# oiwn/toy-heaan-ckks

Measured on AMD Instinct MI355X. Metric: RNS-NTT poly-muls/sec (N=2^16, 16 primes) at 1/2/4/8 GPUs; % HBM roofline, higher is better.
Workload: dtype u32

## Files before the change

toy-heaan-ckks_amd/csrc/rnt_mfma.hip:

```cpp
#include <hip/hip_runtime.h>

#include <vector>

#include "rnt_internal.hpp"
#include "rnt_hostmath.hpp"
#include "rnt_modarith.hpp"
#include "rnt_device.hpp"

namespace rnt {

#ifdef RNT_MF_TRACE
constexpr int kMfTraceWg = 4096, kMfTraceSt = 16;
__device__ uint64_t g_mf_trace[kMfTraceWg * 16 * kMfTraceSt];
#define MF_STAMP(S)                                                                                  \
  do {                                                                                               \
    const uint32_t wg_ = blockIdx.x + blockIdx.y * gridDim.x;                                        \
    if ((threadIdx.x & 63u) == 0 && wg_ < (uint32_t)kMfTraceWg)                                      \
      g_mf_trace[(wg_ * 16 + (threadIdx.x >> 6)) * kMfTraceSt + (S)] = __builtin_amdgcn_s_memrealtime(); \
  } while (0)
#else
#define MF_STAMP(S) \
  do {              \
  } while (0)
#endif

namespace mf {

typedef int v4i __attribute__((ext_vector_type(4)));
constexpr int kT = 1024;
constexpr uint32_t kN = 1u << 16;
constexpr uint32_t K32 = 0x80808080u;

constexpr int S_F1 = 0, S_F2 = 1, S_F3 = 17, S_F4 = 18, S_I4 = 19, S_I3 = 20, S_I2 = 21, S_I1 = 37;
constexpr int kSlots = 38;
constexpr int kMat = 0;
constexpr int kCompF1 = kSlots * 4 * 64;
constexpr int kCompI4 = kCompF1 + 64;
constexpr int kTw3f = kCompI4 + 64;
constexpr int kTw4f = kTw3f + 1024;
constexpr int kTw4i = kTw4f + 16384;
constexpr int kTw3i = kTw4i + 16384;
constexpr int S_F4S = (kTw3i + 1024 + 255) / 256;
#ifndef RNT_MF_FOLD3
#define RNT_MF_FOLD3 1
#endif
#ifndef RNT_MF_FOLD4
#define RNT_MF_FOLD4 0
#endif
constexpr bool kFold3 = RNT_MF_FOLD3 != 0, kFold4 = RNT_MF_FOLD4 != 0;
constexpr int kFoldBase = (S_F4S + 1) * 256;
constexpr int kTwB3 = 1024, kTwB4 = 16384;
constexpr int kTw3fA = kFoldBase, kTw3iA = kTw3fA + 2 * kTwB3;
constexpr int kFold4Base = kFoldBase + (kFold3 ? 4 * kTwB3 : 0);
constexpr int kTw4fA = kFold4Base, kTw4iA = kTw4fA + 2 * kTwB4;
#ifndef RNT_MF_QR
#define RNT_MF_QR 3
#endif
#ifndef RNT_MF_QR_MUL
#define RNT_MF_QR_MUL RNT_MF_QR
#endif
#ifndef RNT_MF_QR_NTT
#define RNT_MF_QR_NTT RNT_MF_QR
#endif
#ifndef RNT_MF_QR_NTTF
#define RNT_MF_QR_NTTF (RNT_MF_QR & 1)
#endif
#ifndef RNT_MF_QR_TENSOR
#define RNT_MF_QR_TENSOR RNT_MF_QR
#endif
constexpr int kQrMul = RNT_MF_QR_MUL & 3, kQrNtt = RNT_MF_QR_NTT & 3, kQrNttFwd = RNT_MF_QR_NTTF & 3;
constexpr int kQrTensor = RNT_MF_QR_TENSOR & 3;
constexpr bool kQrAny = (kQrMul | kQrNtt | kQrNttFwd | kQrTensor) != 0;
constexpr int kQrP4 = 4;
constexpr int kQrBase = kFold4Base + (kFold4 ? 4 * kTwB4 : 0);
static_assert(kQrBase % 256 == 0, "matrix slots are 256 v4i");
constexpr int S_QF1 = kQrBase / 256, S_QF3 = S_QF1 + 1, S_QF4 = S_QF1 + 2, S_QI4 = S_QF1 + 3, S_QI2 = S_QF1 + 4;
constexpr int kQCompF1 = (S_QI2 + 16) * 256, kQCompI4 = kQCompF1 + 128;
constexpr int kQConst = kQCompI4 + 128;
constexpr int kQrEnd = kQConst + 64;
constexpr int kLimb = kQrAny ? kQrEnd : kQrBase;
static_assert(!kQrAny || (kQConst < kLimb && (S_QI2 + 16) * 256 <= kQCompF1), "the plain slots lie inside the limb's table");
#define RNT_MF_QRC "48"
constexpr uint32_t kQrC = 48;
constexpr int kTw3iR = kFold3 ? kTw3iA : kTw3i;
constexpr int kTw4fR = kFold4 ? kTw4fA : kTw4f, kTw4iR = kFold4 ? kTw4iA : kTw4i;
constexpr bool kFold3Fwd = false;
constexpr size_t kLdsBytes = (size_t)160 * 1024;
static_assert(kLdsBytes > 80 * 1024, "one workgroup per CU");

__host__ __device__ constexpr int p3(int c, int i) {
  return 4 * (8 * (i >> 1) + 4 * (i & 1) + 2 * ((c >> 1) & 1) + (c & 1)) + 2 * (c >> 3) + ((c >> 2) & 1);
}
__host__ __device__ constexpr int q2(int c, int i) {
  return p3(8 * (i >> 1) + 4 * (i & 1) + 2 * (c >> 3) + ((c >> 2) & 1), 2 * ((c >> 1) & 1) + (c & 1));
}

struct Mc {
  int32_t q;
  uint32_t nqinv;
  int64_t K;
  int64_t K0;
  int32_t one;
  int32_t s16;
  int32_t mu;
  uint32_t nq, kq, kq0;
};

typedef __amdgpu_buffer_rsrc_t Rsrc;
__device__ __forceinline__ Rsrc rsrc(const void* base, uint32_t bytes) {
  return __builtin_amdgcn_make_buffer_rsrc((void*)base, 0, (int)bytes, 0x00020000);
}
#ifndef RNT_MF_NT
#define RNT_MF_NT 2
#endif
constexpr int kStreamAux = RNT_MF_NT;
#ifndef RNT_MF_LAST_NT
#define RNT_MF_LAST_NT 2
#endif
constexpr int kLastAux = RNT_MF_LAST_NT;
template <int AUX = 0>
__device__ __forceinline__ v4i bld(Rsrc r, uint32_t voff, uint32_t soff) {
  const auto v = __builtin_amdgcn_raw_buffer_load_b128(r, voff, soff, AUX);
  return v4i{(int)v[0], (int)v[1], (int)v[2], (int)v[3]};
}
template <int AUX = 0>
__device__ __forceinline__ void bst(v4i x, Rsrc r, uint32_t voff, uint32_t soff) {
  using V4 = decltype(__builtin_amdgcn_raw_buffer_load_b128(r, 0, 0, 0));
  V4 v;
  v[0] = (uint32_t)x[0];
  v[1] = (uint32_t)x[1];
  v[2] = (uint32_t)x[2];
  v[3] = (uint32_t)x[3];
  __builtin_amdgcn_raw_buffer_store_b128(v, r, voff, soff, AUX);
  asm volatile("s_nop 1" ::"v"(v));
}

template <bool WK>
__device__ __forceinline__ int32_t recomb(int32_t c0, int32_t c1, int32_t c2, int32_t c3, const Mc& m) {
  const int32_t lo = c0 + (int32_t)((uint32_t)c1 << 8);
  const int32_t hi = c2 + (int32_t)((uint32_t)c3 << 8);
  int64_t t;
  if constexpr (WK) {
    uint64_t cc;
    asm("v_mad_i64_i32 %0, %1, %2, 1, %3" : "=v"(t), "=s"(cc) : "v"(lo), "s"(m.K));
  } else {
    t = (int64_t)lo;
  }
  t = (int64_t)hi * m.s16 + t;
  const uint32_t mm = (uint32_t)t * m.nqinv;
  const int64_t v = (int64_t)(int32_t)mm * m.q + t;
  return (int32_t)(v >> 32);
}
template <bool WK>
__device__ __forceinline__ int32_t recomb_q(int32_t c0, int32_t c1, int32_t c2, int32_t c3, const Mc& m) {
  uint32_t lo = (uint32_t)c0 + ((uint32_t)c1 << 8);
  uint32_t hi = (uint32_t)c2 + ((uint32_t)c3 << 8);
  asm("" : "+v"(lo), "+v"(hi));
  uint32_t t = (hi << 16) + lo;
  asm("" : "+v"(t));
  const int32_t qt = __mulhi((int32_t)hi, m.mu);
  return (int32_t)(t + (uint32_t)qt * m.nq + (WK ? m.kq : m.kq0));
}
template <bool QR, bool WK>
__device__ __forceinline__ int32_t recomb_x(int32_t c0, int32_t c1, int32_t c2, int32_t c3, const Mc& m) {
// ... 529 lines not shown
  return (((uint32_t)i << 14) | ((uint32_t)(hc & 1) << 10) | ((uint32_t)(hc >> 1) << 7)) * 4u;
}
__device__ __forceinline__ void load_p1(uint32_t (&x1)[64], Rsrc src, const Th& h) {
  const uint32_t lo = p1_lane(h), wo = p1_wave(h);
#pragma unroll
  for (int hc = 0; hc < 4; ++hc)
#pragma unroll
    for (int i = 0; i < 4; ++i) {
      const v4i v = bld<kStreamAux>(src, lo, wo + p1_reg(i, hc));
#pragma unroll
      for (int e = 0; e < 4; ++e) x1[4 * (4 * hc + e) + i] = (uint32_t)v[e];
    }
}
template <int C0>
__device__ __forceinline__ void ipass_p1(uint32_t (&x1)[64], const v4i (&M)[4], const Mc& m, Rsrc dst,
                                         const Th& h) {
  const v4i z = {0, 0, 0, 0};
#pragma unroll
  for (int c = C0; c < C0 + 8; ++c) {
    v4i b;
#pragma unroll
    for (int i = 0; i < 4; ++i) b[i] = (int)x1[4 * c + i];
    v4i D[4];
    tile<false, false>(D, M, b, z);
#pragma unroll
    for (int i = 0; i < 4; ++i) x1[4 * c + i] = canon(recomb<false>(D[0][i], D[1][i], D[2][i], D[3][i], m), m.q);
    if ((c & 3) == 3) {
      const int hc = c >> 2;
      const uint32_t lo = p1_lane(h), wo = p1_wave(h);
#pragma unroll
      for (int i = 0; i < 4; ++i) {
        v4i v;
#pragma unroll
        for (int e = 0; e < 4; ++e) v[e] = (int)x1[4 * (4 * hc + e) + i];
        bst<kStreamAux>(v, dst, lo, wo + p1_reg(i, hc));
      }
    } else {
      pin4(x1[4 * c + 0], x1[4 * c + 1], x1[4 * c + 2], x1[4 * c + 3]);
    }
    tile_fence();
  }
}

__device__ __forceinline__ uint32_t p4_lane(const Th& h) { return ((h.n() << 4) | (h.g() << 2)) * 4u; }
__device__ __forceinline__ uint32_t p4_soff(const Th& h, int c) { return ((h.w << 12) | ((uint32_t)c << 8)) * 4u; }

struct Tabs {
  Rsrc tab;
  Mc m;
};
__device__ __forceinline__ Tabs tabs_of(const void* mf, const LimbConst<uint32_t>& lc, uint32_t l) {
  Tabs r;
  r.tab = rsrc((const v4i*)mf + (size_t)l * kLimb, (uint32_t)kLimb * 16u);
  r.m.q = (int32_t)lc.q;
  r.m.nqinv = 0u - lc.qinv;
  int64_t K = (int64_t)((uint64_t)K32 << 32), K0 = 0;
  int32_t one = 1, s16 = 65536;
  asm volatile("" : "+s"(one), "+s"(s16), "+s"(K), "+s"(K0));
  if constexpr (kQrAny) {
    int32_t mu = ((const int32_t*)((const v4i*)mf + (size_t)l * kLimb + kQConst))[0];
    uint32_t nq = 0u - lc.q, kq = K32 - (kQrC << 24), kq0 = 0u - (kQrC << 24);
    asm volatile("" : "+s"(mu), "+s"(nq), "+s"(kq), "+s"(kq0));
    r.m.mu = mu;
    r.m.nq = nq;
    r.m.kq = kq;
    r.m.kq0 = kq0;
  }
  r.m.K = K;
  r.m.K0 = K0;
  r.m.one = one;
  r.m.s16 = s16;
  return r;
}

struct NoEpi {
  __device__ void operator()(int, const int32_t (&)[4], uint32_t (&)[64]) const {}
};
template <int NPARK, uint32_t PBASE, uint32_t PSTRIDE>
__device__ __forceinline__ uint32_t park_addr(const uint32_t* lds, const Th& h) {
  static_assert(NPARK * 1024 <= (int)PSTRIDE && PBASE + 16 * PSTRIDE <= kLdsBytes, "park area");
  return (uint32_t)(uintptr_t)lds + PBASE + h.w * PSTRIDE + h.lam() * 16u;
}
template <bool SYNC1, int F4 = S_F4, bool Q4 = false, bool SYNCX = false, int NPARK = 0, uint32_t PBASE = 0,
          uint32_t PSTRIDE = 0, bool F3 = kFold3, int QR = 0, class EPI = NoEpi>
__device__ __forceinline__ void fwd(uint32_t (&x2)[64], Rsrc src, uint32_t* lds, const Th& h, const Tabs& T,
                                    const EPI& epi = EPI{}) {
  const Mc& m = T.m;
  const uint32_t lo = h.lam() * 16u;
  v4i M[4];
  constexpr bool Q1 = (QR & 1) != 0, Q3 = (QR & 2) != 0, Q4P = (QR & kQrP4) != 0;
  load_mat(M, T.tab, Q1 ? S_QF1 : S_F1, lo);
  const v4i comp = bld(T.tab, lo, (uint32_t)(Q1 ? kQCompF1 : kCompF1) * 16u);
  const v4i comp2 = Q1 ? bld(T.tab, lo, (uint32_t)(kQCompF1 + 64) * 16u) : comp;
  uint32_t x1[64];
  load_p1(x1, src, h);
  MF_STAMP(1);
  pass_p1<0, true, Q1>(x1, M, comp, comp2, m);
  MF_STAMP(2);
  if constexpr (SYNC1) __syncthreads();
  uint32_t wb[4], rb[4];
  const uint32_t t3v = h.g() * 256u, t3s = (uint32_t)((F3 ? kTw3fA : kTw3f) + h.w * 64) * 16u;
  if constexpr (Q4) {
    p1_bases4(wb, h);
    x_write_p1q<0>(x1, lds, wb);
    pass_p1<8, true, Q1>(x1, M, comp, comp2, m);
    __syncthreads();
    p2_bases4(rb, h);
    x_read_p2q<0>(x2, lds, rb);
    __syncthreads();
    p1_bases4(wb, h);
    x_write_p1q<1>(x1, lds, wb);
    __syncthreads();
    p2_bases4(rb, h);
    x_read_p2q<1>(x2, lds, rb);
    __syncthreads();
    p1_bases4(wb, h);
    x_write_p1q<2>(x1, lds, wb);
    load_mat(M, T.tab, S_F2 + h.w, lo);
    pass_p2<0, F3>(x2, M, T.tab, t3v, t3s, m);
    __syncthreads();
    p2_bases4(rb, h);
    x_read_p2q<2>(x2, lds, rb);
    __syncthreads();
    p1_bases4(wb, h);
    x_write_p1q<3>(x1, lds, wb);
    __syncthreads();
    p2_bases4(rb, h);
    x_read_p2q<3>(x2, lds, rb);
  } else {
  p1_bases(wb, h);
  x_write_p1<0>(x1, lds, wb);
  pass_p1<8, true, Q1>(x1, M, comp, comp2, m);
  MF_STAMP(3);
  __syncthreads();
  MF_STAMP(4);
  p2_bases(rb, h);
  x_read_p2<0>(x2, lds, rb);
  __syncthreads();
  MF_STAMP(5);
  p1_bases(wb, h);
  x_write_p1<1>(x1, lds, wb);
  load_mat(M, T.tab, S_F2 + h.w, lo);
  pass_p2<0, F3>(x2, M, T.tab, t3v, t3s, m);
  MF_STAMP(6);
  __syncthreads();
  MF_STAMP(7);
  p2_bases(rb, h);
  x_read_p2<1>(x2, lds, rb);
  }
  if constexpr (SYNCX) __syncthreads();
  static_assert(NPARK == 0 || SYNCX, "the park area is free only past SYNCX");
#pragma unroll
  for (int c = 0; c < NPARK; ++c)
    stash_put(park_addr<NPARK, PBASE, PSTRIDE>(lds, h), c, x2[4 * c], x2[4 * c + 1], x2[4 * c + 2], x2[4 * c + 3]);
  pass_p2<8, F3>(x2, M, T.tab, t3v, t3s, m);
  MF_STAMP(8);
#pragma unroll
  for (int c = 0; c < NPARK; ++c) {
    const v4i v = stash_get(park_addr<NPARK, PBASE, PSTRIDE>(lds, h), c);
#pragma unroll
    for (int i = 0; i < 4; ++i) x2[4 * c + i] = (uint32_t)v[i];
  }
  swap_p2p3(x2);
  load_mat(M, T.tab, Q3 ? S_QF3 : S_F3, lo);
  pass_p3<Q3>(x2, M, T.tab, lo, (uint32_t)(kTw4fR + h.w * 1024) * 16u, m);
  MF_STAMP(9);
  load_mat(M, T.tab, F4, lo);
  pass_p4<Q4P>(x2, M, m, epi);
  MF_STAMP(10);
}

template <bool LOAD, bool PK = false, int QR = 0>
__device__ __forceinline__ void inv_x(uint32_t (&x2)[64], Rsrc pr, uint32_t* lds, const Th& h, const Tabs& T) {
  const Mc& m = T.m;
  const uint32_t lo = h.lam() * 16u;
  v4i M[4];
  constexpr bool Q2 = (QR & 1) != 0, Q4 = (QR & 2) != 0;
  load_mat(M, T.tab, Q4 ? S_QI4 : S_I4, lo);
  const v4i comp = bld(T.tab, lo, (uint32_t)(Q4 ? kQCompI4 : kCompI4) * 16u);
  const v4i comp2 = Q4 && !PK ? bld(T.tab, lo, (uint32_t)(kQCompI4 + 64) * 16u) : comp;
  const uint32_t t4s = (uint32_t)(kTw4iR + h.w * 1024) * 16u;
  const v4i tv0 = bld(T.tab, lo, t4s);
  if constexpr (LOAD) {
#pragma unroll
    for (int cc = 0; cc < 16; ++cc) {
      const v4i v = bld<kStreamAux>(pr, p4_lane(h), p4_soff(h, cc));
#pragma unroll
      for (int i = 0; i < 4; ++i) x2[p3(cc, i)] = (uint32_t)v[i];
    }
  } else {
    __syncthreads();
  }
  ipass_p4<PK, Q4>(x2, M, comp, comp2, tv0, T.tab, lo, t4s, m, lds, h);
  load_mat(M, T.tab, S_I3, lo);
  ipass_p3(x2, M, T.tab, h.g() * 16u, (uint32_t)(kTw3iR + h.w * 64) * 16u, m, lds, h);
  swap_q3p2(x2);
  load_mat(M, T.tab, (Q2 ? S_QI2 : S_I2) + h.w, lo);
  uint32_t wb[4], rb[4];
  uint32_t x1[64];
  ipass_p2<0, Q2>(x2, M, m);
  __syncthreads();
  p2_bases(rb, h);
  x_write_p2<0>(x2, lds, rb);
  ipass_p2<8, Q2>(x2, M, m);
  __syncthreads();
  p1_bases(wb, h);
  x_read_p1<0>(x1, lds, wb);
  __syncthreads();
  p2_bases(rb, h);
  x_write_p2<1>(x2, lds, rb);
  load_mat(M, T.tab, S_I1, lo);
  ipass_p1<0>(x1, M, m, pr, h);
  __syncthreads();
  p1_bases(wb, h);
  x_read_p1<1>(x1, lds, wb);
  ipass_p1<8>(x1, M, m, pr, h);
}
__device__ __forceinline__ void inv(Rsrc pr, uint32_t* lds, const Th& h, const Tabs& T) {
  uint32_t x2[64];
  inv_x<true, false, kQrNtt>(x2, pr, lds, h, T);
}

}

template <bool INV>
__global__ void __launch_bounds__(mf::kT, 1)
k_mf_ntt(uint32_t* __restrict__ data, const void* __restrict__ mft, const LimbConst<uint32_t>* __restrict__ lcs,
         uint64_t ls) {
  using namespace mf;
  extern __shared__ __attribute__((aligned(16))) unsigned char smem_raw[];
  uint32_t* lds = (uint32_t*)smem_raw;
  const Th h(threadIdx.x);
  const uint32_t poly = blockIdx.x, l = blockIdx.y;
  MF_STAMP(0);
  uint32_t* p = data + (uint64_t)l * ls + (uint64_t)poly * kN;
  const Tabs T = tabs_of(mft, lcs[l], l);
  const Rsrc pr = rsrc(p, kN * 4u);
  if constexpr (!INV) {
    uint32_t x[64];
    fwd<false, S_F4, false, false, 0, 0, 0, kFold3 && kFold3Fwd, kQrNttFwd>(x, pr, lds, h, T, [&](int cc, const int32_t (&r)[4], uint32_t (&)[64]) {
      bst<kStreamAux>(v4i{(int)canon(r[0], T.m.q), (int)canon(r[1], T.m.q), (int)canon(r[2], T.m.q), (int)canon(r[3], T.m.q)}, pr,
          p4_lane(h), p4_soff(h, cc));
    });
  } else {
    inv(pr, lds, h, T);
  }
#ifdef RNT_MF_TRACE
  __builtin_amdgcn_s_waitcnt(0);
  MF_STAMP(11);
#endif
}

__global__ void __launch_bounds__(mf::kT, 1)
k_mf_tensor(uint32_t* __restrict__ d0, uint32_t* __restrict__ d1, uint32_t* __restrict__ d2, uint64_t ols,
            const uint32_t* __restrict__ c0, const uint32_t* __restrict__ c1, const uint32_t* __restrict__ c0p,
            const uint32_t* __restrict__ c1p, uint64_t ils, uint32_t* __restrict__ scratch, uint32_t slots,
            const void* __restrict__ mft, const LimbConst<uint32_t>* __restrict__ lcs,
            uint32_t* __restrict__ d2hat) {
  using namespace mf;
  extern __shared__ __attribute__((aligned(16))) unsigned char smem_raw[];
  uint32_t* lds = (uint32_t*)smem_raw;
  const Th h(threadIdx.x);
  const uint32_t poly = blockIdx.x, l = blockIdx.y;
  const uint64_t oo = (uint64_t)l * ols + (uint64_t)poly * kN, io = (uint64_t)l * ils + (uint64_t)poly * kN;
  const LimbConst<uint32_t> lc = lcs[l];
  const Tabs T = tabs_of(mft, lc, l);
  const uint32_t q = lc.q, nqi = T.m.nqinv;
  uint64_t so;
  if (slots) {
    const uint32_t xcc = __builtin_amdgcn_s_getreg((31 << 11) | 20) & 7u;
    const uint32_t cu = (__builtin_amdgcn_s_getreg((31 << 11) | 4) >> 8) & 0xffu;
    so = (uint64_t)((xcc << 8) | cu) << 16;
  } else {
    so = (uint64_t)(poly + l * gridDim.x) << 16;
  }
  const Rsrc R0 = rsrc(d0 + oo, kN * 4u), R1 = rsrc(d1 + oo, kN * 4u), R2 = rsrc(d2 + oo, kN * 4u);
  const Rsrc RS = rsrc(scratch + so, kN * 4u);
  const bool want_hat = d2hat != nullptr;
  const Rsrc RH = rsrc(want_hat ? d2hat + oo : d2 + oo, kN * 4u);
  const uint32_t pl = p4_lane(h);
  auto canon4 = [q](const int32_t (&r)[4]) {
    return v4i{(int)canon(r[0], (int32_t)q), (int)canon(r[1], (int32_t)q), (int)canon(r[2], (int32_t)q),
               (int)canon(r[3], (int32_t)q)};
  };
  auto mmul = [q, nqi](uint32_t a, uint32_t b) {
    const uint64_t t = (uint64_t)a * b;
    const uint32_t mm = (uint32_t)t * nqi;
    const uint32_t r = (uint32_t)((t + (uint64_t)mm * q) >> 32);
    return r >= q ? r - q : r;
  };
  const uint32_t rm = lc.rmod, rmp = lc.rmod_p;
  uint32_t x[64];
  constexpr bool SX = RNT_MF_TENSOR_SYNCX != 0;
  constexpr int NP = SX ? RNT_MF_TENSOR_PARK : 0;
  constexpr uint32_t PB = 128u * 1024u, PS = 2048u;
  constexpr int MEAS = RNT_MF_TENSOR_MEAS;
  fwd<false, S_F4, false, SX, NP, PB, PS, kFold3, kQrTensor>(x, rsrc(c0 + io, kN * 4u), lds, h, T, [&](int cc, const int32_t (&r)[4], uint32_t (&)[64]) {
    if constexpr (MEAS != 3) bst(canon4(r), R1, pl, p4_soff(h, cc));
  });
  fwd<!SX, S_F4, false, SX, NP, PB, PS, kFold3, kQrTensor>(x, rsrc(c1 + io, kN * 4u), lds, h, T, [&](int cc, const int32_t (&r)[4], uint32_t (&)[64]) {
    if constexpr (MEAS != 1) bst(canon4(r), RS, pl, p4_soff(h, cc));
  });
  fwd<!SX, S_F4, false, SX, NP, PB, PS, kFold3, kQrTensor>(x, rsrc(c0p + io, kN * 4u), lds, h, T, [&](int cc, const int32_t (&r)[4], uint32_t (&)[64]) {
    const v4i a0 = MEAS == 3 ? canon4(r) : bld(R1, pl, p4_soff(h, cc));
    const v4i a1 = MEAS == 1 ? canon4(r) : bld(RS, pl, p4_soff(h, cc));
    const v4i b = canon4(r);
    v4i o0, t;
#pragma unroll
    for (int i = 0; i < 4; ++i) {
      o0[i] = (int)mmul((uint32_t)a0[i], (uint32_t)b[i]);
      t[i] = (int)mmul((uint32_t)a1[i], (uint32_t)b[i]);
    }
    bst<kLastAux>(o0, R0, pl, p4_soff(h, cc));
    if constexpr (MEAS != 2) bst(t, R2, pl, p4_soff(h, cc));
  });
  fwd<!SX, S_F4, false, RNT_MF_TENSOR_PARK4 && SX, RNT_MF_TENSOR_PARK4 ? NP : 0, PB, PS, kFold3, kQrTensor>(x, rsrc(c1p + io, kN * 4u), lds, h, T, [&](int cc, const int32_t (&r)[4], uint32_t (&xx)[64]) {
    const v4i b = canon4(r);
    const v4i a0 = MEAS == 3 ? b : bld<kLastAux>(R1, pl, p4_soff(h, cc));
    const v4i a1 = MEAS == 1 ? b : bld<kLastAux>(RS, pl, p4_soff(h, cc));
    const v4i t = MEAS == 2 ? b : bld<kLastAux>(R2, pl, p4_soff(h, cc));
    v4i o1;
#pragma unroll
    for (int i = 0; i < 4; ++i) {
      const uint32_t s = (uint32_t)t[i] + mmul((uint32_t)a0[i], (uint32_t)b[i]);
      o1[i] = (int)(s >= q ? s - q : s);
      const uint32_t m = mmul((uint32_t)a1[i], (uint32_t)b[i]);
      const uint32_t qh = (uint32_t)(((uint64_t)m * rmp) >> 32);
      const uint32_t v = m * rm - qh * q;
      xx[p3(cc, i)] = v >= q ? v - q : v;
    }
    pin4(xx[p3(cc, 0)], xx[p3(cc, 1)], xx[p3(cc, 2)], xx[p3(cc, 3)]);
    bst<kLastAux>(o1, R1, pl, p4_soff(h, cc));
    if (want_hat)
      bst<kLastAux>(v4i{(int)xx[p3(cc, 0)], (int)xx[p3(cc, 1)], (int)xx[p3(cc, 2)], (int)xx[p3(cc, 3)]}, RH, pl,
                    p4_soff(h, cc));
  });
  inv_x<false, false, kQrTensor>(x, R2, lds, h, T);
}

#ifndef RNT_MF_MUL_Q4
#define RNT_MF_MUL_Q4 1
#endif
#ifndef RNT_MF_MUL_NOSYNC1
#define RNT_MF_MUL_NOSYNC1 1
#endif
#ifndef RNT_MF_MUL_PARK
#define RNT_MF_MUL_PARK 4
#endif
#ifndef RNT_MF_MUL_MEAS
#define RNT_MF_MUL_MEAS 0
#endif
#ifndef RNT_MF_SLOT_ST_AUX
#define RNT_MF_SLOT_ST_AUX 0
#endif
#ifndef RNT_MF_MUL_MEAS_SKIP
#define RNT_MF_MUL_MEAS_SKIP (RNT_MF_MUL_MEAS ? 16 - kMulLdsTiles : 0)
#endif
constexpr int kMulLdsTiles = RNT_MF_MUL_Q4 ? 6 : 2;
constexpr uint32_t kMulLdsBase = RNT_MF_MUL_Q4 ? (1u << 14) : (1u << 15);
static_assert(kMulLdsBase * 4 + (size_t)kMulLdsTiles * 16 * 1024 <= mf::kLdsBytes, "in the LDS");
__global__ void __launch_bounds__(mf::kT, 1)
k_mf_mul(uint32_t* c, const uint32_t* a, const uint32_t* b, uint64_t ls, uint32_t* __restrict__ scratch,
         uint32_t slots, const void* __restrict__ mft, const LimbConst<uint32_t>* __restrict__ lcs) {
  using namespace mf;
  extern __shared__ __attribute__((aligned(16))) unsigned char smem_raw[];
  uint32_t* lds = (uint32_t*)smem_raw;
  const Th h(threadIdx.x);
  const uint32_t poly = blockIdx.x, l = blockIdx.y;
  const uint64_t o = (uint64_t)l * ls + (uint64_t)poly * kN;
  const LimbConst<uint32_t> lc = lcs[l];
  const Tabs T = tabs_of(mft, lc, l);
  uint64_t so;
  if (slots) {
    const uint32_t xcc = __builtin_amdgcn_s_getreg((31 << 11) | 20) & 7u;
    const uint32_t cu = (__builtin_amdgcn_s_getreg((31 << 11) | 4) >> 8) & 0xffu;
    so = (uint64_t)((xcc << 8) | cu) << 16;
  } else {
    so = (uint64_t)(poly + l * gridDim.x) << 16;
  }
  const Rsrc RS = rsrc(scratch + so, kN * 4u);
  uint32_t x[64];
  auto hat = [&](int t) -> v4i& { return ((v4i*)(lds + kMulLdsBase) + h.w * (kMulLdsTiles * 64) + h.lam())[t * 64]; };
  constexpr int NP = RNT_MF_MUL_Q4 ? RNT_MF_MUL_PARK : 0;
  constexpr int QM = kQrMul | ((kQrMul & 1) ? kQrP4 : 0);
  constexpr int FA = (kQrMul & 1) ? S_F4 : S_F4S, FB = (kQrMul & 1) ? S_QF4 : S_F4;
  fwd<false, FA, false, RNT_MF_MUL_Q4 != 0, NP, kMulLdsBase * 4, kMulLdsTiles * 1024, kFold3, QM>(x, rsrc(a + o, kN * 4u), lds, h, T, [&](int cc, const int32_t (&r)[4], uint32_t (&)[64]) {
    if (cc >= 16 - kMulLdsTiles)
      hat(cc - (16 - kMulLdsTiles)) = v4i{r[0], r[1], r[2], r[3]};
    else if (cc >= RNT_MF_MUL_MEAS_SKIP)
      bst<RNT_MF_SLOT_ST_AUX>(v4i{r[0], r[1], r[2], r[3]}, RS, p4_lane(h), p4_soff(h, cc));
  });
  fwd<!(RNT_MF_MUL_Q4 && RNT_MF_MUL_NOSYNC1), FB, RNT_MF_MUL_Q4 != 0, (NP > 0), NP, 0, 4096, kFold3, QM>(x, rsrc(b + o, kN * 4u), lds, h, T, [&](int cc, const int32_t (&r)[4], uint32_t (&xx)[64]) {
    const v4i ah = cc >= 16 - kMulLdsTiles ? hat(cc - (16 - kMulLdsTiles))
                   : cc < RNT_MF_MUL_MEAS_SKIP ? v4i{r[0], r[1], r[2], r[3]} : bld(RS, p4_lane(h), p4_soff(h, cc));
#pragma unroll
    for (int i = 0; i < 4; ++i) {
      xx[p3(cc, i)] = (uint32_t)mont<true>(ah[i], r[i], T.m) ^ K32;
    }
    pin4(xx[p3(cc, 0)], xx[p3(cc, 1)], xx[p3(cc, 2)], xx[p3(cc, 3)]);
  });
  inv_x<false, true, kQrMul>(x, rsrc(c + o, kN * 4u), lds, h, T);
}

namespace {
using host::brv;
using host::invmod;
using host::mulmod;
using host::powmod;

int32_t centred(uint64_t v, uint64_t q) {
  v %= q;
  return v > q / 2 ? (int32_t)((int64_t)v - (int64_t)q) : (int32_t)v;
}

void expand(const uint64_t (&W)[16][16], uint64_t q, uint64_t R, bool DA, int KAP, int32_t* out) {
  int32_t E[16][16][4];
  for (int o = 0; o < 16; ++o)
    for (int k = 0; k < 16; ++k)
      for (int b = 0; b < 4; ++b) E[o][k][b] = centred(mulmod(mulmod(W[o][k], (1ull << (8 * b)) % q, q), R, q), q);
  for (int a = 0; a < 4; ++a)
    for (int lam = 0; lam < 64; ++lam)
      for (int i = 0; i < 4; ++i) {
        const int g = lam >> 4, r = lam & 15;
        const int kin = KAP ? 4 * g + i : 4 * i + g;
        const int jout = DA ? r : (KAP ? r : 4 * (r & 3) + (r >> 2));
        uint32_t wd = 0;
        for (int b = 0; b < 4; ++b) {
          const uint32_t u = (uint32_t)E[jout][kin][b] + 0x80808080u;
          wd |= ((((u >> (8 * a)) & 0xFFu) ^ 0x80u) & 0xFFu) << (8 * b);
        }
        out[(a * 64 + lam) * 4 + i] = (int32_t)wd;
      }
}

}

int mf_build(Tables* t, std::string* err) {
  using namespace mf;
  const size_t L = t->L;
  const uint64_t n = kN;
  std::vector<int32_t> all((size_t)L * kLimb * 4);
  std::vector<uint64_t> tw(n), itw(n), pw(n), ipw(n);
  for (size_t l = 0; l < L; ++l) {
    const uint64_t q = t->moduli[l], psi = t->psi[l], psinv = invmod(psi, q);
    uint64_t x = 1, y = 1;
    for (uint64_t j = 0; j < n; ++j) {
      pw[j] = x;
      ipw[j] = y;
      x = mulmod(x, psi, q);
      y = mulmod(y, psinv, q);
    }
    for (uint64_t g = 0; g < n; ++g) {
      tw[g] = pw[brv(g, 16)];
      itw[g] = ipw[brv(g, 16)];
    }
    const uint64_t R = (uint64_t)(((host::u128)1 << 32) % q);
    {
      const double rb = (double)q / 2 + 16384.0;
      if (rb * rb / 4294967296.0 + (double)q / 2 + 1 >= (double)0x7F7F7F7Fu) {
        *err = "MFMA tables: the product bound exceeds the packed digit range for this prime";
        return -1;
      }
      if ((kFold3 || kFold4) &&
          (268435456.0 + 1048576.0) * (double)q / 4294967296.0 + (double)q / 2 + 1 >= (double)0x7F7F7F7Fu) {
        *err = "MFMA tables: the folded twist bound exceeds the packed digit range for this prime";
        return -1;
      }
    }
    if (kQrAny) {
      const uint64_t Bq = (1ull << 28) + (1ull << 20) + (1ull << 15), c8 = (uint64_t)kQrC << 8, c24 = (uint64_t)kQrC << 24;
      const uint64_t mu = (1ull << 48) / q, rho = (1ull << 48) % q;
      const uint64_t neg = Bq + c24 + (((Bq - c8) * rho) >> 32) + 1;
      const int64_t pos = (int64_t)(Bq + q + (((Bq + c8) * rho) >> 32) + 1) - (int64_t)c24;
      const uint64_t rq = pos > (int64_t)neg ? (uint64_t)pos : neg, lim = 0x7F7F7F7Full;
      const bool ok = mu <= 0x7FFFFFFFull && rq <= lim &&
                      (host::u128)rq * q / ((host::u128)1 << 33) + q / 2 + 1 < lim &&
                      (host::u128)rq * rq / ((host::u128)1 << 32) + q / 2 + 1 < lim;
      if (!ok) {
        *err = "MFMA tables: the quotient-estimate reduction's bound exceeds the packed digit range for this prime";
        return -1;
      }
    }
    uint64_t M0[16][16];
    for (int k = 0; k < 16; ++k) {
// ... 58 lines not shown
      expand(F, q, 1, false, 1, slot(S_QF4));
      expand(Fi, q, 1, true, 1, slot(S_QI4));
      for (int U = 0; U < 16; ++U) {
        const uint64_t bei = itw[128 + 8 * U];
        for (int k = 0; k < 16; ++k)
          for (int j = 0; j < 16; ++j) W[k][j] = mulmod(powmod(bei, (uint64_t)k, q), Fi[k][j], q);
        expand(W, q, 1, false, 0, slot(S_QI2 + U));
      }
      lt[(size_t)kQConst * 4] = (int32_t)(uint32_t)((1ull << 48) / q);
    }
    const uint64_t bias = mulmod(R, (1ull << 30) % q, q);
    {
      int32_t cf[16], ci[16];
      for (int j = 0; j < 16; ++j) {
        uint64_t s0 = 0, s1 = 0;
        for (int k = 0; k < 16; ++k) {
          s0 = (s0 + M0[j][k]) % q;
          s1 = (s1 + Fi[j][k]) % q;
        }
        cf[j] = centred(mulmod(bias, s0, q), q);
        ci[j] = centred(mulmod(bias, s1, q), q);
      }
      int32_t* c1 = lt + (size_t)kCompF1 * 4;
      int32_t* c4 = lt + (size_t)kCompI4 * 4;
      for (int lam = 0; lam < 64; ++lam)
        for (int i = 0; i < 4; ++i) {
          c1[lam * 4 + i] = cf[4 * i + (lam >> 4)];
          c4[lam * 4 + i] = ci[lam & 15];
        }
      if (kQrAny) {
        const uint64_t pb = (1ull << 30) % q;
        int32_t* q1 = lt + (size_t)kQCompF1 * 4;
        int32_t* q4 = lt + (size_t)kQCompI4 * 4;
        auto split = [](int32_t v, int32_t* v0, int32_t* v2) {
          *v2 = (v + 32768) >> 16;
          *v0 = v - *v2 * 65536;
        };
        for (int j = 0; j < 16; ++j) {
          uint64_t s0 = 0, s1 = 0;
          for (int k = 0; k < 16; ++k) {
            s0 = (s0 + M0[j][k]) % q;
            s1 = (s1 + Fi[j][k]) % q;
          }
          cf[j] = centred(mulmod(pb, s0, q), q);
          ci[j] = centred(mulmod(pb, s1, q), q);
        }
        for (int lam = 0; lam < 64; ++lam)
          for (int i = 0; i < 4; ++i) {
            split(cf[4 * i + (lam >> 4)], &q1[lam * 4 + i], &q1[(64 + lam) * 4 + i]);
            split(ci[lam & 15], &q4[lam * 4 + i], &q4[(64 + lam) * 4 + i]);
          }
      }
    }
    const uint64_t s16 = (1ull << 16) % q;
    auto put = [&](int32_t* tab, bool fold, int dist, size_t idx, uint64_t tv) {
      if (fold) {
        tab[idx] = centred(tv, q);
        tab[(size_t)dist * 4 + idx] = centred(mulmod(tv, s16, q), q);
      } else {
        tab[idx] = centred(mulmod(tv, R, q), q);
      }
    };
    int32_t* t3f = lt + (size_t)kTw3f * 4;
    int32_t* t3fa = lt + (size_t)kTw3fA * 4;
    int32_t* t3i = lt + (size_t)kTw3iR * 4;
    for (int w = 0; w < 16; ++w)
      for (int g = 0; g < 4; ++g)
        for (int c = 0; c < 16; ++c)
          for (int i = 0; i < 4; ++i) {
            const int U3 = (w << 4) | (i << 2) | g;
            const uint64_t tv = powmod(tw[2048 + 8 * U3], (uint64_t)c, q);
            put(t3f, false, 0, ((w * 4 + g) * 16 + c) * 4 + i, tv);
            if (kFold3) put(t3fa, true, kTwB3, ((w * 4 + g) * 16 + c) * 4 + i, tv);
          }
    for (int w = 0; w < 16; ++w)
      for (int c = 0; c < 16; ++c)
        for (int g = 0; g < 4; ++g)
          for (int i = 0; i < 4; ++i) {
            const int U3 = (w << 4) | c;
            put(t3i, kFold3, kTwB3, ((w * 16 + c) * 4 + g) * 4 + i, powmod(itw[2048 + 8 * U3], (uint64_t)(4 * g + i), q));
          }
    int32_t* t4f = lt + (size_t)kTw4fR * 4;
    int32_t* t4i = lt + (size_t)kTw4iR * 4;
    for (int w = 0; w < 16; ++w)
      for (int c = 0; c < 16; ++c)
        for (int lam = 0; lam < 64; ++lam)
          for (int i = 0; i < 4; ++i) {
            const int g = lam >> 4, nn = lam & 15;
            const int Uf = (w << 8) | (c << 4) | nn;
            put(t4f, kFold4, kTwB4, ((w * 16 + c) * 64 + lam) * 4 + i, powmod(tw[32768 + 8 * Uf], (uint64_t)(4 * g + i), q));
            const int Ui = (w << 8) | (c << 4) | (4 * g + i);
            put(t4i, kFold4, kTwB4, ((w * 16 + c) * 64 + lam) * 4 + i, powmod(itw[32768 + 8 * Ui], (uint64_t)nn, q));
          }
  }
  const size_t bytes = all.size() * sizeof(int32_t);
  void* dev = nullptr;
  if (hipError_t e = hipMalloc(&dev, bytes); e != hipSuccess) {
    *err = std::string("hipMalloc(MFMA tables): ") + hipGetErrorString(e);
    return -3;
  }
  if (hipError_t e = hipMemcpy(dev, all.data(), bytes, hipMemcpyHostToDevice); e != hipSuccess) {
    (void)hipFree(dev);
    *err = std::string("hipMemcpy(MFMA tables): ") + hipGetErrorString(e);
    return -2;
  }
  t->mf = dev;
  return 0;
}

static hipError_t launch_ntt_t(const Launch& k, const void* fn, void* data, uint64_t ls) {
  hipError_t e = hipFuncSetAttribute(fn, hipFuncAttributeMaxDynamicSharedMemorySize, (int)mf::kLdsBytes);
  if (e != hipSuccess) return e;
  uint32_t* d = (uint32_t*)data;
  const void* mft = (const mf::v4i*)k.t->mf + (size_t)k.tab0 * mf::kLimb;
  const LimbConst<uint32_t>* lcs = (const LimbConst<uint32_t>*)k.t->lconst + k.tab0;
  void* args[] = {&d, &mft, &lcs, &ls};
  return hipLaunchKernel(fn, dim3((unsigned)k.B, (unsigned)k.L), dim3(mf::kT), args, mf::kLdsBytes, k.s);
}

hipError_t launch_mf_tensor(const Launch& k, void* d0, void* d1, void* d2, uint64_t ols, const void* c0,
                            const void* c1, const void* c0p, const void* c1p, uint64_t ils, void* scratch) {
  if (k.B == 0 || k.L == 0) return hipSuccess;
  if (k.B > 0x7fffffffull || k.L > 65535) return hipErrorInvalidConfiguration;
  const void* fn = (const void*)k_mf_tensor;
  hipError_t e = hipFuncSetAttribute(fn, hipFuncAttributeMaxDynamicSharedMemorySize, (int)mf::kLdsBytes);
  if (e != hipSuccess) return e;
  uint32_t slots = (uint64_t)k.B * k.L >= kPlaneSlots ? 1u : 0u;
  const void* mft = k.t->mf;
  const LimbConst<uint32_t>* lcs = (const LimbConst<uint32_t>*)k.t->lconst;
  void* d2hat = k.d2hat;
  void* args[] = {&d0, &d1, &d2, &ols, &c0, &c1, &c0p, &c1p, &ils, &scratch, &slots, &mft, &lcs, &d2hat};
  return hipLaunchKernel(fn, dim3((unsigned)k.B, (unsigned)k.L), dim3(mf::kT), args, mf::kLdsBytes, k.s);
}

hipError_t launch_mf_mul(const Launch& k, void* c, const void* a, const void* b, uint64_t ls, void* scratch) {
  if (k.B == 0 || k.L == 0) return hipSuccess;
  if (k.B > 0x7fffffffull || k.L > 65535) return hipErrorInvalidConfiguration;
  const void* fn = (const void*)k_mf_mul;
  hipError_t e = hipFuncSetAttribute(fn, hipFuncAttributeMaxDynamicSharedMemorySize, (int)mf::kLdsBytes);
  if (e != hipSuccess) return e;
  uint32_t slots = (uint64_t)k.B * k.L >= kPlaneSlots ? 1u : 0u;
  const void* mft = k.t->mf;
  const LimbConst<uint32_t>* lcs = (const LimbConst<uint32_t>*)k.t->lconst;
  void* args[] = {&c, &a, &b, &ls, &scratch, &slots, &mft, &lcs};
  return hipLaunchKernel(fn, dim3((unsigned)k.B, (unsigned)k.L), dim3(mf::kT), args, mf::kLdsBytes, k.s);
}

#ifdef RNT_MF_TRACE
extern "C" __attribute__((visibility("default"))) int rnt_debug_mf_trace(uint64_t* out) {
  return (int)hipMemcpyFromSymbol(out, HIP_SYMBOL(g_mf_trace), sizeof(g_mf_trace));
}
#endif

hipError_t launch_mf_ntt(const Launch& k, int inverse, void* data, uint64_t ls) {
  if (k.B == 0 || k.L == 0) return hipSuccess;
  if (k.B > 0x7fffffffull || k.L > 65535) return hipErrorInvalidConfiguration;
  return inverse ? launch_ntt_t(k, (const void*)k_mf_ntt<true>, data, ls)
                 : launch_ntt_t(k, (const void*)k_mf_ntt<false>, data, ls);
}

}
```

Measured before the change: 171,000.

## Split pass-3/4 twiddles into per-wave matrix factor and shared residual table

Factors the per-wave part of the stage-4 twiddle into per-wave pass-4 MFMA matrices (forward and inverse, with matching compensation constants), leaving a small wave-independent residual twist table shared by all waves. Pass 3 and inverse pass 4 then read a 1024-entry table instead of a per-wave 16×1024 one, which is meant to cut table-memory traffic and cache footprint. It is enabled by default for NTT, forward NTT and tensor paths (split mask 14), but not for poly-mul. The cost is extra per-wave matrix slots in the table, a larger per-limb table, and host-side verification that the factorisation multiplies back to the original twiddles.

```diff
diff --git a/toy-heaan-ckks_amd/csrc/rnt_mfma.hip b/toy-heaan-ckks_amd/csrc/rnt_mfma.hip
--- a/toy-heaan-ckks_amd/csrc/rnt_mfma.hip
+++ b/toy-heaan-ckks_amd/csrc/rnt_mfma.hip
@@ -78,8 +78,23 @@
 constexpr int kQCompF1 = (S_QI2 + 16) * 256, kQCompI4 = kQCompF1 + 128;
 constexpr int kQConst = kQCompI4 + 128;
 constexpr int kQrEnd = kQConst + 64;
-constexpr int kLimb = kQrAny ? kQrEnd : kQrBase;
-static_assert(!kQrAny || (kQConst < kLimb && (S_QI2 + 16) * 256 <= kQCompF1), "the plain slots lie inside the limb's table");
+constexpr int kQrLimb = kQrAny ? kQrEnd : kQrBase;
+static_assert(!kQrAny || (kQConst < kQrLimb && (S_QI2 + 16) * 256 <= kQCompF1), "the plain slots lie inside the limb's table");
+#ifndef RNT_MF_SPLIT
+#define RNT_MF_SPLIT 14
+#endif
+constexpr int kSplit = RNT_MF_SPLIT & 15;
+constexpr bool kSpMul = (kSplit & 1) != 0, kSpNtt = (kSplit & 2) != 0, kSpNttFwd = (kSplit & 4) != 0;
+constexpr bool kSpTensor = (kSplit & 8) != 0;
+constexpr bool kSpAny = kSplit != 0, kSpAll = kSplit == 15;
+static_assert(!(kSpAny && kFold4), "the split twist keeps pass_p3 / ipass_p4 in two steps");
+constexpr int S_WF4 = (kQrLimb + 255) / 256, S_WF4S = S_WF4 + 16, S_WQF4 = S_WF4 + 32, S_WI4 = S_WF4 + 48, S_WQI4 = S_WF4 + 64;
+constexpr int kTwR4f = (S_WQI4 + 16) * 256;
+constexpr int kTwR4i = kTwR4f + 1024;
+constexpr int kCompI4W = kTwR4i + 1024;
+constexpr int kQCompI4W = kCompI4W + 1024;
+constexpr int kLimb = kSpAny ? kQCompI4W + 2048 : kQrLimb;
+constexpr int sp_f4(int f4) { return f4 == S_F4 ? S_WF4 : f4 == S_F4S ? S_WF4S : S_WQF4; }
 #define RNT_MF_QRC "48"
 constexpr uint32_t kQrC = 48;
 constexpr int kTw3iR = kFold3 ? kTw3iA : kTw3i;
@@ -775,7 +790,7 @@
   return (uint32_t)(uintptr_t)lds + PBASE + h.w * PSTRIDE + h.lam() * 16u;
 }
 template <bool SYNC1, int F4 = S_F4, bool Q4 = false, bool SYNCX = false, int NPARK = 0, uint32_t PBASE = 0,
-          uint32_t PSTRIDE = 0, bool F3 = kFold3, int QR = 0, class EPI = NoEpi>
+          uint32_t PSTRIDE = 0, bool F3 = kFold3, int QR = 0, bool SP = false, class EPI = NoEpi>
 __device__ __forceinline__ void fwd(uint32_t (&x2)[64], Rsrc src, uint32_t* lds, const Th& h, const Tabs& T,
                                     const EPI& epi = EPI{}) {
   const Mc& m = T.m;
@@ -856,23 +871,26 @@
   }
   swap_p2p3(x2);
   load_mat(M, T.tab, Q3 ? S_QF3 : S_F3, lo);
-  pass_p3<Q3>(x2, M, T.tab, lo, (uint32_t)(kTw4fR + h.w * 1024) * 16u, m);
+  static_assert(F4 == S_F4 || F4 == S_F4S || F4 == S_QF4, "a last forward matrix");
+  pass_p3<Q3>(x2, M, T.tab, lo, SP ? (uint32_t)kTwR4f * 16u : (uint32_t)(kTw4fR + h.w * 1024) * 16u, m);
   MF_STAMP(9);
-  load_mat(M, T.tab, F4, lo);
+  load_mat(M, T.tab, SP ? sp_f4(F4) + h.w : (uint32_t)F4, lo);
   pass_p4<Q4P>(x2, M, m, epi);
   MF_STAMP(10);
 }
 
-template <bool LOAD, bool PK = false, int QR = 0>
+template <bool LOAD, bool PK = false, int QR = 0, bool SP = false>
 __device__ __forceinline__ void inv_x(uint32_t (&x2)[64], Rsrc pr, uint32_t* lds, const Th& h, const Tabs& T) {
   const Mc& m = T.m;
   const uint32_t lo = h.lam() * 16u;
   v4i M[4];
   constexpr bool Q2 = (QR & 1) != 0, Q4 = (QR & 2) != 0;
-  load_mat(M, T.tab, Q4 ? S_QI4 : S_I4, lo);
-  const v4i comp = bld(T.tab, lo, (uint32_t)(Q4 ? kQCompI4 : kCompI4) * 16u);
-  const v4i comp2 = Q4 && !PK ? bld(T.tab, lo, (uint32_t)(kQCompI4 + 64) * 16u) : comp;
-  const uint32_t t4s = (uint32_t)(kTw4iR + h.w * 1024) * 16u;
+  load_mat(M, T.tab, SP ? (Q4 ? S_WQI4 : S_WI4) + h.w : (uint32_t)(Q4 ? S_QI4 : S_I4), lo);
+  const uint32_t cs = SP ? (uint32_t)(Q4 ? kQCompI4W + h.w * 128 : kCompI4W + h.w * 64) * 16u
+                         : (uint32_t)(Q4 ? kQCompI4 : kCompI4) * 16u;
+  const v4i comp = bld(T.tab, lo, cs);
+  const v4i comp2 = Q4 && !PK ? bld(T.tab, lo, cs + 64u * 16u) : comp;
+  const uint32_t t4s = SP ? (uint32_t)kTwR4i * 16u : (uint32_t)(kTw4iR + h.w * 1024) * 16u;
   const v4i tv0 = bld(T.tab, lo, t4s);
   if constexpr (LOAD) {
 #pragma unroll
@@ -911,7 +929,7 @@
 }
 __device__ __forceinline__ void inv(Rsrc pr, uint32_t* lds, const Th& h, const Tabs& T) {
   uint32_t x2[64];
-  inv_x<true, false, kQrNtt>(x2, pr, lds, h, T);
+  inv_x<true, false, kQrNtt, kSpNtt>(x2, pr, lds, h, T);
 }
 
 }
@@ -931,7 +949,7 @@
   const Rsrc pr = rsrc(p, kN * 4u);
   if constexpr (!INV) {
     uint32_t x[64];
-    fwd<false, S_F4, false, false, 0, 0, 0, kFold3 && kFold3Fwd, kQrNttFwd>(x, pr, lds, h, T, [&](int cc, const int32_t (&r)[4], uint32_t (&)[64]) {
+    fwd<false, S_F4, false, false, 0, 0, 0, kFold3 && kFold3Fwd, kQrNttFwd, kSpNttFwd>(x, pr, lds, h, T, [&](int cc, const int32_t (&r)[4], uint32_t (&)[64]) {
       bst<kStreamAux>(v4i{(int)canon(r[0], T.m.q), (int)canon(r[1], T.m.q), (int)canon(r[2], T.m.q), (int)canon(r[3], T.m.q)}, pr,
           p4_lane(h), p4_soff(h, cc));
     });
@@ -988,13 +1006,13 @@
   constexpr int NP = SX ? RNT_MF_TENSOR_PARK : 0;
   constexpr uint32_t PB = 128u * 1024u, PS = 2048u;
   constexpr int MEAS = RNT_MF_TENSOR_MEAS;
-  fwd<false, S_F4, false, SX, NP, PB, PS, kFold3, kQrTensor>(x, rsrc(c0 + io, kN * 4u), lds, h, T, [&](int cc, const int32_t (&r)[4], uint32_t (&)[64]) {
+  fwd<false, S_F4, false, SX, NP, PB, PS, kFold3, kQrTensor, kSpTensor>(x, rsrc(c0 + io, kN * 4u), lds, h, T, [&](int cc, const int32_t (&r)[4], uint32_t (&)[64]) {
     if constexpr (MEAS != 3) bst(canon4(r), R1, pl, p4_soff(h, cc));
   });
-  fwd<!SX, S_F4, false, SX, NP, PB, PS, kFold3, kQrTensor>(x, rsrc(c1 + io, kN * 4u), lds, h, T, [&](int cc, const int32_t (&r)[4], uint32_t (&)[64]) {
+  fwd<!SX, S_F4, false, SX, NP, PB, PS, kFold3, kQrTensor, kSpTensor>(x, rsrc(c1 + io, kN * 4u), lds, h, T, [&](int cc, const int32_t (&r)[4], uint32_t (&)[64]) {
     if constexpr (MEAS != 1) bst(canon4(r), RS, pl, p4_soff(h, cc));
   });
-  fwd<!SX, S_F4, false, SX, NP, PB, PS, kFold3, kQrTensor>(x, rsrc(c0p + io, kN * 4u), lds, h, T, [&](int cc, const int32_t (&r)[4], uint32_t (&)[64]) {
+  fwd<!SX, S_F4, false, SX, NP, PB, PS, kFold3, kQrTensor, kSpTensor>(x, rsrc(c0p + io, kN * 4u), lds, h, T, [&](int cc, const int32_t (&r)[4], uint32_t (&)[64]) {
     const v4i a0 = MEAS == 3 ? canon4(r) : bld(R1, pl, p4_soff(h, cc));
     const v4i a1 = MEAS == 1 ? canon4(r) : bld(RS, pl, p4_soff(h, cc));
     const v4i b = canon4(r);
@@ -1007,7 +1025,7 @@
     bst<kLastAux>(o0, R0, pl, p4_soff(h, cc));
     if constexpr (MEAS != 2) bst(t, R2, pl, p4_soff(h, cc));
   });
-  fwd<!SX, S_F4, false, RNT_MF_TENSOR_PARK4 && SX, RNT_MF_TENSOR_PARK4 ? NP : 0, PB, PS, kFold3, kQrTensor>(x, rsrc(c1p + io, kN * 4u), lds, h, T, [&](int cc, const int32_t (&r)[4], uint32_t (&xx)[64]) {
+  fwd<!SX, S_F4, false, RNT_MF_TENSOR_PARK4 && SX, RNT_MF_TENSOR_PARK4 ? NP : 0, PB, PS, kFold3, kQrTensor, kSpTensor>(x, rsrc(c1p + io, kN * 4u), lds, h, T, [&](int cc, const int32_t (&r)[4], uint32_t (&xx)[64]) {
     const v4i b = canon4(r);
     const v4i a0 = MEAS == 3 ? b : bld<kLastAux>(R1, pl, p4_soff(h, cc));
     const v4i a1 = MEAS == 1 ? b : bld<kLastAux>(RS, pl, p4_soff(h, cc));
@@ -1028,7 +1046,7 @@
       bst<kLastAux>(v4i{(int)xx[p3(cc, 0)], (int)xx[p3(cc, 1)], (int)xx[p3(cc, 2)], (int)xx[p3(cc, 3)]}, RH, pl,
                     p4_soff(h, cc));
   });
-  inv_x<false, false, kQrTensor>(x, R2, lds, h, T);
+  inv_x<false, false, kQrTensor, kSpTensor>(x, R2, lds, h, T);
 }
 
 #ifndef RNT_MF_MUL_Q4
@@ -1077,13 +1095,13 @@
   constexpr int NP = RNT_MF_MUL_Q4 ? RNT_MF_MUL_PARK : 0;
   constexpr int QM = kQrMul | ((kQrMul & 1) ? kQrP4 : 0);
   constexpr int FA = (kQrMul & 1) ? S_F4 : S_F4S, FB = (kQrMul & 1) ? S_QF4 : S_F4;
-  fwd<false, FA, false, RNT_MF_MUL_Q4 != 0, NP, kMulLdsBase * 4, kMulLdsTiles * 1024, kFold3, QM>(x, rsrc(a + o, kN * 4u), lds, h, T, [&](int cc, const int32_t (&r)[4], uint32_t (&)[64]) {
+  fwd<false, FA, false, RNT_MF_MUL_Q4 != 0, NP, kMulLdsBase * 4, kMulLdsTiles * 1024, kFold3, QM, kSpMul>(x, rsrc(a + o, kN * 4u), lds, h, T, [&](int cc, const int32_t (&r)[4], uint32_t (&)[64]) {
     if (cc >= 16 - kMulLdsTiles)
       hat(cc - (16 - kMulLdsTiles)) = v4i{r[0], r[1], r[2], r[3]};
     else if (cc >= RNT_MF_MUL_MEAS_SKIP)
       bst<RNT_MF_SLOT_ST_AUX>(v4i{r[0], r[1], r[2], r[3]}, RS, p4_lane(h), p4_soff(h, cc));
   });
-  fwd<!(RNT_MF_MUL_Q4 && RNT_MF_MUL_NOSYNC1), FB, RNT_MF_MUL_Q4 != 0, (NP > 0), NP, 0, 4096, kFold3, QM>(x, rsrc(b + o, kN * 4u), lds, h, T, [&](int cc, const int32_t (&r)[4], uint32_t (&xx)[64]) {
+  fwd<!(RNT_MF_MUL_Q4 && RNT_MF_MUL_NOSYNC1), FB, RNT_MF_MUL_Q4 != 0, (NP > 0), NP, 0, 4096, kFold3, QM, kSpMul>(x, rsrc(b + o, kN * 4u), lds, h, T, [&](int cc, const int32_t (&r)[4], uint32_t (&xx)[64]) {
     const v4i ah = cc >= 16 - kMulLdsTiles ? hat(cc - (16 - kMulLdsTiles))
                    : cc < RNT_MF_MUL_MEAS_SKIP ? v4i{r[0], r[1], r[2], r[3]} : bld(RS, p4_lane(h), p4_soff(h, cc));
 #pragma unroll
@@ -1092,7 +1110,7 @@
     }
     pin4(xx[p3(cc, 0)], xx[p3(cc, 1)], xx[p3(cc, 2)], xx[p3(cc, 3)]);
   });
-  inv_x<false, true, kQrMul>(x, rsrc(c + o, kN * 4u), lds, h, T);
+  inv_x<false, true, kQrMul, kSpMul>(x, rsrc(c + o, kN * 4u), lds, h, T);
 }
 
 namespace {
@@ -1317,16 +1335,67 @@
           }
     int32_t* t4f = lt + (size_t)kTw4fR * 4;
     int32_t* t4i = lt + (size_t)kTw4iR * 4;
+    int32_t* r4f = lt + (size_t)kTwR4f * 4;
+    int32_t* r4i = lt + (size_t)kTwR4i * 4;
+    uint64_t wf[16][16], wi[16][16];
     for (int w = 0; w < 16; ++w)
-      for (int c = 0; c < 16; ++c)
-        for (int lam = 0; lam < 64; ++lam)
-          for (int i = 0; i < 4; ++i) {
-            const int g = lam >> 4, nn = lam & 15;
-            const int Uf = (w << 8) | (c << 4) | nn;
-            put(t4f, kFold4, kTwB4, ((w * 16 + c) * 64 + lam) * 4 + i, powmod(tw[32768 + 8 * Uf], (uint64_t)(4 * g + i), q));
-            const int Ui = (w << 8) | (c << 4) | (4 * g + i);
-            put(t4i, kFold4, kTwB4, ((w * 16 + c) * 64 + lam) * 4 + i, powmod(itw[32768 + 8 * Ui], (uint64_t)nn, q));
+      for (int k = 0; k < 16; ++k) {
+        wf[w][k] = powmod(tw[32768 + 2048 * w], (uint64_t)k, q);
+        wi[w][k] = powmod(itw[32768 + 2048 * w], (uint64_t)k, q);
+      }
+    for (int c = 0; c < 16; ++c)
+      for (int lam = 0; lam < 64; ++lam)
+        for (int i = 0; i < 4; ++i) {
+          const int g = lam >> 4, nn = lam & 15, k = 4 * g + i;
+          const uint64_t rf = powmod(mulmod(tw[32768 + 8 * ((c << 4) | nn)], itw[32768], q), (uint64_t)k, q);
+          const uint64_t ri = powmod(mulmod(itw[32768 + 8 * ((c << 4) | k)], tw[32768], q), (uint64_t)nn, q);
+          if (kSpAny) {
+            put(r4f, false, 0, (c * 64 + lam) * 4 + i, rf);
+            put(r4i, false, 0, (c * 64 + lam) * 4 + i, ri);
           }
+          for (int w = 0; w < 16; ++w) {
+            const uint64_t tf = powmod(tw[32768 + 8 * ((w << 8) | (c << 4) | nn)], (uint64_t)k, q);
+            const uint64_t ti = powmod(itw[32768 + 8 * ((w << 8) | (c << 4) | k)], (uint64_t)nn, q);
+            if (kSpAny && (mulmod(wf[w][k], rf, q) != tf || mulmod(wi[w][nn], ri, q) != ti)) {
+              *err = "MFMA tables: the split pass-3 twist does not multiply back to the whole one";
+              return -1;
+            }
+            if (!kSpAll) {
+              put(t4f, kFold4, kTwB4, ((w * 16 + c) * 64 + lam) * 4 + i, tf);
+              put(t4i, kFold4, kTwB4, ((w * 16 + c) * 64 + lam) * 4 + i, ti);
+            }
+          }
+        }
+    if (kSpAny) {
+      const uint64_t pb = (1ull << 30) % q;
+      for (int w = 0; w < 16; ++w) {
+        for (int j = 0; j < 16; ++j)
+          for (int k = 0; k < 16; ++k) W[j][k] = mulmod(F[j][k], wf[w][k], q);
+        expand(W, q, R, false, 1, slot(S_WF4 + w));
+        if (kQrAny) expand(W, q, 1, false, 1, slot(S_WQF4 + w));
+        for (int j = 0; j < 16; ++j)
+          for (int k = 0; k < 16; ++k) W[j][k] = mulmod(W[j][k], R, q);
+        expand(W, q, R, false, 1, slot(S_WF4S + w));
+        for (int k = 0; k < 16; ++k)
+          for (int j = 0; j < 16; ++j) W[k][j] = mulmod(wi[w][k], Fi[k][j], q);
+        expand(W, q, R, true, 1, slot(S_WI4 + w));
+        if (kQrAny) expand(W, q, 1, true, 1, slot(S_WQI4 + w));
+        int32_t* c4 = lt + (size_t)(kCompI4W + w * 64) * 4;
+        int32_t* q4 = lt + (size_t)(kQCompI4W + w * 128) * 4;
+        for (int j = 0; j < 16; ++j) {
+          uint64_t s1 = 0;
+          for (int k = 0; k < 16; ++k) s1 = (s1 + W[j][k]) % q;
+          const int32_t cm = centred(mulmod(bias, s1, q), q), cp = centred(mulmod(pb, s1, q), q);
+          const int32_t v2 = (cp + 32768) >> 16, v0 = cp - v2 * 65536;
+          for (int lam = j; lam < 64; lam += 16)
+            for (int i = 0; i < 4; ++i) {
+              c4[lam * 4 + i] = cm;
+              q4[lam * 4 + i] = v0;
+              q4[(64 + lam) * 4 + i] = v2;
+            }
+        }
+      }
+    }
   }
   const size_t bytes = all.size() * sizeof(int32_t);
   void* dev = nullptr;
```

Result: no change. 169,700 (median of 2 runs) (-0.7%).
